# StefanDenn3r/Unsupervised_Anomaly_Detection_Brain_MRI

Measured on AMD Instinct MI355X. Metric: MRI slices/sec VAE train step (128x128, bs=64), higher is better.
Workload: dtype bf16x3; 1 GPU; BASELINE.json configs[1]: VAE 128x128x1 slices, batch 64 per GPU, fwd + bwd + TF-Adam (lr 1e-4, beta1 0.5), dropout 0.2, inter_res 8, zDim 128; global_batch=64, per_gpu_batch=64, parallelism=single

## Files before the change

include/uad_hip.h:

```cpp
#ifndef UAD_HIP_H
#define UAD_HIP_H

#include <stddef.h>
#include <stdint.h>

#ifdef __cplusplus
extern "C" {
#endif
#pragma GCC visibility push(default)

enum { UAD_OK = 0, UAD_ERR_INVALID = 1, UAD_ERR_HIP = 2, UAD_ERR_UNSUPPORTED = 3 };
enum { UAD_ARCH_AE = 0, UAD_ARCH_VAE = 1, UAD_ARCH_CEVAE = 2, UAD_ARCH_GMVAE_SPATIAL = 3,
       UAD_ARCH_AE_SPATIAL = 4 };
enum { UAD_BUF_PARAMS = 0, UAD_BUF_GRADS = 1, UAD_BUF_ADAM_M = 2, UAD_BUF_ADAM_V = 3 };
enum { UAD_SEG_DECODER = 0, UAD_SEG_BOTTLENECK = 1, UAD_SEG_ENCODER = 2, UAD_SEG_ENCODER_HI = 3, UAD_SEG_ENCODER_LO = 4, UAD_SEG_ALL = -1 };
enum { UAD_MATH_F32 = 0, UAD_MATH_BF16X3 = 1,
       UAD_MATH_BF16X3_ALL = 2 };
enum { UAD_MATH_BF16X6 = 3 };

typedef struct uad_model uad_model_t;

typedef struct {
    int arch;
    int height;
// ... 235 lines not shown
int uad_op_conv_w(const uad_conv_desc_t* d, const float* big, const uad_xform_t* xfb, const float* small_,
                  const uad_xform_t* xfs, float* dW, void* stream);
enum { UAD_OP_EPI_BIAS = 0, UAD_OP_EPI_BWD_ACT = 1, UAD_OP_EPI_FINAL = 2, UAD_OP_EPI_FINAL_TRAIN = 3, UAD_OP_EPI_FINAL_DC = 4 };
enum { UAD_OP_XF_IN = 1, UAD_OP_XF_SMALL = 2, UAD_OP_XF_FINAL_BWD = 4 };
int uad_op_conv_plan(const uad_conv_desc_t* d, int kind, int epi, int xf_flags, long long* out);
int uad_op_conv_d_final(const uad_conv_desc_t* d, const float* small_in, const uad_xform_t* xf, const float* W, const float* bias, const uad_xform_t* bn,
                        const float* wf, const float* bf, const float* x, float inv_batch, float* x_hat, float* l1, float* rec_sum,
                        unsigned* bits, float* dxhat, float* dc, float* red, void* stream);
int uad_op_conv_f_final_bwd(const uad_conv_desc_t* d, const unsigned* bits, const float* dxhat, const float* wf, const uad_xform_t* bn, const float* W,
                            const float* bias, const float* mul, const float* add, float* small_out, void* stream);
int uad_op_conv_first_fwd(const uad_conv_desc_t* d, const float* x, const float* W, const float* bias, float* out,
                          void* stream);
int uad_op_conv_first_wgrad(const uad_conv_desc_t* d, const float* x, const float* g, float* dW, void* stream);
int uad_op_adam(float* p, const float* g, float* m, float* v, long long n, float lr_t, float beta1, float beta2,
                float eps, float gscale, void* stream);

#pragma GCC visibility pop
#ifdef __cplusplus
}
#endif
#endif
```

unsupervised_anomaly_detection_brain_mri_amd/_lib.py:

```python
import ctypes as C
import os

_HERE = os.path.dirname(os.path.abspath(__file__))
LIB_PATH = os.environ.get('UAD_LIB') or os.path.join(_HERE, 'libuad_hip.so')

UAD_OK = 0
ARCH_AE, ARCH_VAE, ARCH_CEVAE, ARCH_GMVAE_SPATIAL, ARCH_AE_SPATIAL = 0, 1, 2, 3, 4
BUF_PARAMS, BUF_GRADS, BUF_ADAM_M, BUF_ADAM_V = 0, 1, 2, 3
SEG_DECODER, SEG_BOTTLENECK, SEG_ENCODER, SEG_ENCODER_HI, SEG_ENCODER_LO, SEG_ALL = 0, 1, 2, 3, 4, -1
MATH_F32, MATH_BF16X3, MATH_BF16X3_ALL, MATH_BF16X6 = 0, 1, 2, 3

c_float_p = C.c_void_p


class UadConfig(C.Structure):
    _fields_ = [('arch', C.c_int), ('height', C.c_int), ('width', C.c_int), ('channels', C.c_int),
                ('inter_res', C.c_int), ('zdim', C.c_int), ('max_batch', C.c_int),
                ('dim_c', C.c_int), ('dim_z', C.c_int), ('dim_w', C.c_int), ('c_lambda', C.c_float)]


class UadRngJob(C.Structure):
    _fields_ = [('out', C.c_void_p), ('per_sample', C.c_int), ('kind', C.c_int), ('rate', C.c_float), ('stream', C.c_int)]


# ... 31 lines not shown
HISTOGRAM_MAX_CLASSES, HISTOGRAM_SUM_CHAIN = 4, 1073
GAN_ENCODER, GAN_GENERATOR, GAN_DISCRIMINATOR = 0, 1, 2
GAN_UNIFIED, GAN_RESNET, GAN_ANOVAEGAN, GAN_AAE = 0, 1, 2, 3
GAN_GROUP_VAE = 3
BUF_ADAM_M2, BUF_ADAM_V2 = 4, 5
GAN_SCALARS = ('gen_loss', 'disc_fake', 'disc_real', 'penalty', 'disc_loss', 'loss_img', 'loss_fts', 'enc_loss',
               'reconstructionLoss', 'kl', 'gm_loss', 'gm_con', 'gm_w', 'gm_c')


class UadConvDesc(C.Structure):
    _fields_ = [(k, C.c_int) for k in ('N', 'HB', 'WB', 'CB', 'HS', 'WS', 'CS', 'KS', 'S', 'P')]


class UadXform(C.Structure):
    _fields_ = [('scale', C.c_void_p), ('shift', C.c_void_p), ('alpha', C.c_float)]


SYMBOLS = {
    'uad_last_error': (C.c_char_p, []),
    'uad_version': (C.c_char_p, []),
    'uad_create': (C.c_int, [C.POINTER(UadConfig), C.POINTER(C.c_void_p)]),
    'uad_destroy': (C.c_int, [C.c_void_p]),
    'uad_param_count': (C.c_longlong, [C.c_void_p]),
    'uad_num_tensors': (C.c_int, [C.c_void_p]),
    'uad_tensor_info': (C.c_int, [C.c_void_p, C.c_int, C.c_char_p, C.c_int, C.POINTER(C.c_longlong),
                                  C.POINTER(C.c_int), C.POINTER(C.c_int)]),
    'uad_buffer': (C.c_void_p, [C.c_void_p, C.c_int]),
    'uad_grad_segment': (C.c_int, [C.c_void_p, C.c_int, C.POINTER(C.c_longlong), C.POINTER(C.c_longlong)]),
    'uad_set_params': (C.c_int, [C.c_void_p, C.c_void_p, C.c_longlong]),
    'uad_get_params': (C.c_int, [C.c_void_p, C.c_void_p, C.c_longlong]),
# ... 103 lines not shown
    'uad_op_conv_d_bwdact': (C.c_int, [C.POINTER(UadConvDesc), C.c_void_p, C.c_void_p, C.c_void_p,
                                       C.POINTER(UadXform), C.c_void_p, C.c_void_p, C.c_void_p, C.c_void_p]),
    'uad_op_conv_w': (C.c_int, [C.POINTER(UadConvDesc), C.c_void_p, C.POINTER(UadXform), C.c_void_p,
                                C.POINTER(UadXform), C.c_void_p, C.c_void_p]),
    'uad_op_conv_plan': (C.c_int, [C.POINTER(UadConvDesc), C.c_int, C.c_int, C.c_int, C.POINTER(C.c_longlong)]),
    'uad_op_conv_d_final': (C.c_int, [C.POINTER(UadConvDesc), C.c_void_p, C.POINTER(UadXform), C.c_void_p, C.c_void_p, C.POINTER(UadXform),
                                      C.c_void_p, C.c_void_p, C.c_void_p, C.c_float, C.c_void_p, C.c_void_p, C.c_void_p,
                                      C.c_void_p, C.c_void_p, C.c_void_p, C.c_void_p, C.c_void_p]),
    'uad_op_conv_f_final_bwd': (C.c_int, [C.POINTER(UadConvDesc), C.c_void_p, C.c_void_p, C.c_void_p, C.POINTER(UadXform), C.c_void_p,
                                          C.c_void_p, C.c_void_p, C.c_void_p, C.c_void_p, C.c_void_p]),
    'uad_op_conv_first_fwd': (C.c_int, [C.POINTER(UadConvDesc), C.c_void_p, C.c_void_p, C.c_void_p, C.c_void_p,
                                        C.c_void_p]),
    'uad_op_conv_first_wgrad': (C.c_int, [C.POINTER(UadConvDesc), C.c_void_p, C.c_void_p, C.c_void_p, C.c_void_p]),
    'uad_op_adam': (C.c_int, [C.c_void_p, C.c_void_p, C.c_void_p, C.c_void_p, C.c_longlong, C.c_float, C.c_float,
                              C.c_float, C.c_float, C.c_float, C.c_void_p]),
}

_lib = None


def load():
    global _lib
    if _lib is not None:
        return _lib
    if not os.path.exists(LIB_PATH):
        raise RuntimeError(
            f'{LIB_PATH} is missing: the HIP extension has not been built '
            f'(run `python -m unsupervised_anomaly_detection_brain_mri_amd.build` or __graft_entry__.build()). '
            f'There is no CPU fallback.')
    import torch
# ... 16 lines not shown
```

unsupervised_anomaly_detection_brain_mri_amd/csrc/uad_conv_plan.hip:

```cpp
#include <stdint.h>
#include <stdio.h>
#include <stdlib.h>
#include <string.h>
#include "uad_conv_launch.h"
#include "uad_conv_k3_plan.h"

namespace {
thread_local bool g_any_order_next = false;
thread_local bool g_any_order_w_next = false;
inline bool take_request(bool& flag) { const bool on = flag; flag = false; return on; }

struct SpatialChoice { bool ok; int TH, TW, BN, CK; };
inline SpatialChoice choose_spatial(const UadConvDesc& d, int CA, int Nn, bool f_type = true) {
    SpatialChoice c{false, 0, 0, 0, 0};
    if (!(d.KS == 5 && d.S == 2 && d.P == 1)) return c;
    if (d.HB != 2 * d.HS || d.WB != 2 * d.WS) return c;
    if (CA > XF_LDS_CH) return c;
    if (Nn % 64 == 0 && CA % 32 == 0 && d.HS % 8 == 0 && d.WS % 8 == 0) { c = SpatialChoice{true, 8, 8, 64, 32}; return c; }
    if (Nn % 32 == 0 && CA % 16 == 0 && d.HS % 8 == 0 && d.WS % 16 == 0) {
        c = SpatialChoice{true, 8, 16, 32, (!f_type && CA % 32 == 0) ? 32 : 16};
        return c;
    }
    return c;
}
// ... 382 lines not shown
    a.lws = ilog2_exact(d.WS); a.lhs = ilog2_exact(d.HS); a.dbgbuf = nullptr;
    dim3 grid((a.Mtot + c.BM - 1) / c.BM, (d.CS + c.BN - 1) / c.BN, c.splits);
    static const bool w16_ok = !getenv("UAD_NO_W16");
    const bool w16 = generic_bf16x3 && w16_ok && !xfb.scale && !xfs.scale && c.BN == 64 && d.CB % 4 == 0 && d.CS % 4 == 0;
    uad_gemm_launch_w(a, grid, c.BM, c.BN, w16, st);
    if (c.splits > 1 && !defer_reduce) uad_launch_reduce_partials(partial, c.splits, a.Mtot * d.CS, 1.0f, dW, hop());
}

void uad_conv_any_order_next(bool on) { g_any_order_next = on; }
void uad_conv_w_any_order_next(bool on) { g_any_order_w_next = on; }
void uad_launch_conv_w_reduce(const UadConvDesc& d, float* dW, float* partial, hipStream_t st, bool math_bf16x3) {
    const W5Choice w5 = choose_w5(d, math_bf16x3);
    const int splits = w5.ok ? w5.splits : choose_w(d).splits;
    if (splits > 1) uad_launch_reduce_partials(partial, splits, d.KS * d.KS * d.CB * d.CS, 1.0f, dW, st);
}

void uad_conv_w_plan_query(const UadConvDesc& d, bool math_bf16x3, int planes16, bool fbb, bool xa, bool xs, bool generic_bf16x3, bool defer_reduce, long long* out) {
    const long long slab = (long long)d.KS * d.KS * d.CB * d.CS;
    out[5] = -1; out[6] = -1; out[9] = 0;
    const W5Choice w5 = choose_w5(d, math_bf16x3);
    if (w5.ok) {
        const bool use16 = w5_use16(math_bf16x3, planes16, fbb, xa, xs);
        out[0] = 1; out[1] = w5.splits; out[2] = (w5.total_tiles % w5.tiles_per_split) ? 1 : 0; out[3] = w5_ncsb(d, use16); out[4] = w5.total_tiles;
        if (math_bf16x3 && planes16 == 3) out[5] = use16 ? 1 : 0;
        out[7] = w5.tiles_per_split; out[8] = w5.splits > 1 ? w5.splits * slab : 0;
        return;
    }
    const WK3Choice k3 = choose_wk3(d);
    if (wk3_takes(k3, math_bf16x3 || generic_bf16x3, planes16, defer_reduce, fbb || xa || xs)) {
        out[0] = 2; out[1] = k3.splits; out[2] = (k3.total_tiles % k3.tiles_per_split) ? 1 : 0; out[3] = 0; out[4] = k3.total_tiles;
// ... 9 lines not shown
```

unsupervised_anomaly_detection_brain_mri_amd/csrc/uad_kernels.h:

```cpp
#pragma once
#include <stdint.h>
#ifndef UAD_HOST_EMULATION
#include <hip/hip_runtime.h>

int uad_fail(int code, const char* fmt, ...);
#define HIP_TRY(expr)                                                                                      \
    do {                                                                                                   \
        hipError_t e_ = (expr);                                                                            \
        if (e_ != hipSuccess) return uad_fail(UAD_ERR_HIP, "%s failed: %s", #expr, hipGetErrorString(e_)); \
    } while (0)

struct UadConvDesc {
    int N;
    int HB, WB, CB;
    int HS, WS, CS;
    int KS, S, P;
};

struct UadXform {
    const float* scale = nullptr;
    const float* shift = nullptr;
    float alpha = 1.f;
    float mult = 1.f;
    const float* fb_dxhat = nullptr;
// ... 63 lines not shown
bool uad_conv_d_x6_form_ok(const UadEpilogue& ep, bool has_xf);
void uad_conv_w_plan_query(const UadConvDesc& d, bool math_bf16x3, int planes16, bool fbb, bool xa, bool xs, bool generic_bf16x3, bool defer_reduce, long long* out);
size_t uad_conv_w_partial_floats(const UadConvDesc& d);
bool uad_conv_w_supports_fb_bits(const UadConvDesc& d, bool math_bf16x3);
void uad_launch_conv_w(const UadConvDesc& d, const float* big, UadXform xfb, const float* small, UadXform xfs,
                       float* dW, float* partial, hipStream_t st, bool math_bf16x3 = false,
                       hipStream_t reduce_st = nullptr, hipEvent_t ev = nullptr, bool generic_bf16x3 = false, bool defer_reduce = false, int planes16 = 2);
void uad_launch_conv_w_reduce(const UadConvDesc& d, float* dW, float* partial, hipStream_t st, bool math_bf16x3);

void uad_launch_reduce_partials(const float* partial, int S, int L, float scale, float* out, hipStream_t st);
void uad_launch_bn_grad_finalize(const float* colpart, int T, int C, const float* gamma, float rstd,
                                 float* dgamma, float* dbeta, float* dbias, hipStream_t st, float* scratch = nullptr);
size_t uad_bn_grad_finalize_scratch_floats(int C);
void uad_launch_final_gradfin(const float* red, int C, const float* gamma, float rstd, float* dwf, float* dbf, float* dgamma, float* dbeta,
                              float* dbias, hipStream_t st);
constexpr size_t kUadColsumScratchFloats = 64 * 1024;
void uad_launch_colsum(const float* g, int rows, int C, float* out, float* scratch, hipStream_t st);
size_t uad_colsum_scratch_floats(int rows, int C);

void uad_launch_conv_first_fwd(const UadConvDesc& d, const float* x, const float* W, const float* bias,
                               float* out, hipStream_t st);
size_t uad_conv_first_wgrad_partial_floats(const UadConvDesc& d);
void uad_launch_conv_first_wgrad(const UadConvDesc& d, const float* x, const float* g, float* dW,
                                 float* partial, hipStream_t st);

struct UadFinalArgs {
    int N, H, W, C;
    const float* c_last;
    const float* scale;
    const float* shift;
// ... 175 lines not shown
```

unsupervised_anomaly_detection_brain_mri_amd/csrc/uad_misc.hip:

```cpp
#include "uad_kernels.h"
#include <stdint.h>

namespace {

__device__ __forceinline__ float wave_sum(float v) {
#pragma unroll
    for (int o = 32; o > 0; o >>= 1) v += __shfl_xor(v, o);
    return v;
}

typedef float v4f_nt __attribute__((ext_vector_type(4)));
template <int JL, int SL>
__global__ void __launch_bounds__(JL * SL) reduce_partials4_kernel(const float* __restrict__ partial, int S, int L, float scale, float* __restrict__ out) {
    __shared__ v4f_nt red[SL][JL];
    const int jl = threadIdx.x % JL, sl = threadIdx.x / JL;
    const int j4 = blockIdx.x * JL + jl, L4 = L >> 2;
    v4f_nt a0 = {0.f, 0.f, 0.f, 0.f}, a1 = a0, a2 = a0, a3 = a0;
    if (j4 < L4) {
        const v4f_nt* p = reinterpret_cast<const v4f_nt*>(partial) + j4;
        int s = sl;
        for (; s + 3 * SL < S; s += 4 * SL) {
            const v4f_nt v0 = __builtin_nontemporal_load(p + (size_t)s * L4), v1 = __builtin_nontemporal_load(p + (size_t)(s + SL) * L4);
            const v4f_nt v2 = __builtin_nontemporal_load(p + (size_t)(s + 2 * SL) * L4), v3 = __builtin_nontemporal_load(p + (size_t)(s + 3 * SL) * L4);
            a0 += v0; a1 += v1; a2 += v2; a3 += v3;
        }
        for (; s < S; s += SL) a0 += __builtin_nontemporal_load(p + (size_t)s * L4);
    }
    red[sl][jl] = (a0 + a1) + (a2 + a3);
    __syncthreads();
    if (sl == 0 && j4 < L4) {
        v4f_nt t = red[0][jl];
#pragma unroll
        for (int k = 1; k < SL; ++k) t += red[k][jl];
        reinterpret_cast<v4f_nt*>(out)[j4] = t * scale;
    }
}

template <int SL>
__global__ void __launch_bounds__(64 * SL) reduce_partials_kernel(const float* __restrict__ partial, int S, int L,
                                                                  float scale, float* __restrict__ out, int nt) {
    __shared__ float red[SL][64];
    const int jl = threadIdx.x & 63, sl = threadIdx.x >> 6;
    const int j = blockIdx.x * 64 + jl;
    float a0 = 0.f, a1 = 0.f, a2 = 0.f, a3 = 0.f;
    if (j < L) {
        int s = sl;
        if (nt) {
            for (; s + 3 * SL < S; s += 4 * SL) {
                a0 += __builtin_nontemporal_load(partial + (size_t)s * L + j);
                a1 += __builtin_nontemporal_load(partial + (size_t)(s + SL) * L + j);
                a2 += __builtin_nontemporal_load(partial + (size_t)(s + 2 * SL) * L + j);
                a3 += __builtin_nontemporal_load(partial + (size_t)(s + 3 * SL) * L + j);
            }
        }
        for (; s + 3 * SL < S; s += 4 * SL) {
            a0 += partial[(size_t)s * L + j];
            a1 += partial[(size_t)(s + SL) * L + j];
            a2 += partial[(size_t)(s + 2 * SL) * L + j];
            a3 += partial[(size_t)(s + 3 * SL) * L + j];
        }
        for (; s < S; s += SL) a0 += partial[(size_t)s * L + j];
    }
    red[sl][jl] = (a0 + a1) + (a2 + a3);
    __syncthreads();
    if (sl == 0 && j < L) {
        float t = 0.f;
#pragma unroll
        for (int k = 0; k < SL; ++k) t += red[k][jl];
        out[j] = t * scale;
    }
}

__global__ void __launch_bounds__(1024) bn_grad_finalize_kernel(const float* __restrict__ colpart, int T, int C,
                                                                const float* __restrict__ gamma, float rstd,
                                                                float* __restrict__ dgamma, float* __restrict__ dbeta,
                                                                float* __restrict__ dbias) {
    __shared__ float red[2][32][33];
    const int cl = threadIdx.x & 31, g = threadIdx.x >> 5;
    const int c = blockIdx.x * 32 + cl;
    float s1 = 0.f, s2 = 0.f;
    if (c < C) {
        for (int t = g; t < T; t += 32) {
            s1 += colpart[((size_t)t * 2 + 0) * C + c];
            s2 += colpart[((size_t)t * 2 + 1) * C + c];
        }
// ... 54 lines not shown
        if (dbias) dbias[c] = gamma[c] * rstd * a1;
    }
}

__global__ void __launch_bounds__(256) final_gradfin_kernel(const float* __restrict__ red, int C, const float* __restrict__ gamma, float rstd,
                                                            float* __restrict__ dwf, float* __restrict__ dbf, float* __restrict__ dgamma,
                                                            float* __restrict__ dbeta, float* __restrict__ dbias) {
    for (int c = threadIdx.x; c < C; c += 256) {
        const float s1 = red[C + c], s2 = red[2 * C + c];
        dwf[c] = red[c];
        if (dbeta) dbeta[c] = s1;
        if (dgamma) dgamma[c] = s2 * rstd;
        if (dbias) dbias[c] = gamma[c] * rstd * s1;
    }
    if (threadIdx.x == 0) dbf[0] = red[3 * C];
}

__global__ void __launch_bounds__(256) colsum_kernel(const float* __restrict__ g, int rows, int C, int rows_per_chunk,
                                                     float* __restrict__ out) {
    __shared__ float red[8][33];
    const int cl = threadIdx.x & 31, rl = threadIdx.x >> 5;
    const int c = blockIdx.x * 32 + cl;
    const int r0 = blockIdx.y * rows_per_chunk;
    const int r1 = min(r0 + rows_per_chunk, rows);
    float s = 0.f;
    if (c < C)
        for (int r = r0 + rl; r < r1; r += 8) s += g[(size_t)r * C + c];
    red[rl][cl] = s;
    __syncthreads();
    if (rl == 0 && c < C) {
// ... 758 lines not shown
}
void uad_launch_clock_probe(unsigned long long* out, unsigned long long ticks, hipStream_t st) {
    hipLaunchKernelGGL(clock_probe_kernel, dim3(1), dim3(64), 0, st, out, ticks);
}

void uad_launch_gather_slices(const float* src, const int* idx, int n, long long slice_elems, float* out, hipStream_t st) {
    const long long f4 = slice_elems / 4;
    int bx = (int)((f4 + 255) / 256); if (bx > 64) bx = 64; if (bx < 1) bx = 1;
    hipLaunchKernelGGL(gather_slices_kernel, dim3(bx, n), dim3(256), 0, st, src, idx, f4, out);
}
void uad_launch_gather_mask(const unsigned char* labels, const int* idx, int n, long long slice_px, const unsigned char* lut,
                            float* out, hipStream_t st) {
    int bx = (int)((slice_px + 255) / 256); if (bx > 64) bx = 64; if (bx < 1) bx = 1;
    hipLaunchKernelGGL(gather_mask_kernel, dim3(bx, n), dim3(256), 0, st, labels, idx, slice_px, lut, out);
}
void uad_launch_reduce_partials(const float* partial, int S, int L, float scale, float* out, hipStream_t st) {
    const int blocks = (L + 63) / 64;
    constexpr int nt = 1;
    static const bool r4 = getenv("UAD_NO_REDUCE4") == nullptr;
    if (r4 && S > 8 && L % 4 == 0 && L >= 1024 && ((uintptr_t)partial & 15) == 0 && ((uintptr_t)out & 15) == 0) {
        const int L4 = L / 4;
        if ((L4 + 63) / 64 >= 256) hipLaunchKernelGGL((reduce_partials4_kernel<64, 8>), dim3((L4 + 63) / 64), dim3(512), 0, st, partial, S, L, scale, out);
        else if ((L4 + 31) / 32 >= 256) hipLaunchKernelGGL((reduce_partials4_kernel<32, 16>), dim3((L4 + 31) / 32), dim3(512), 0, st, partial, S, L, scale, out);
        else hipLaunchKernelGGL((reduce_partials4_kernel<16, 32>), dim3((L4 + 15) / 16), dim3(512), 0, st, partial, S, L, scale, out);
        return;
    }
    if (blocks >= 256 || S <= 8)
        hipLaunchKernelGGL((reduce_partials_kernel<4>), dim3(blocks), dim3(256), 0, st, partial, S, L, scale, out, nt);
    else
        hipLaunchKernelGGL((reduce_partials_kernel<16>), dim3(blocks), dim3(1024), 0, st, partial, S, L, scale, out, nt);
}

void uad_launch_final_gradfin(const float* red, int C, const float* gamma, float rstd, float* dwf, float* dbf, float* dgamma, float* dbeta,
                              float* dbias, hipStream_t st) {
    hipLaunchKernelGGL(final_gradfin_kernel, dim3(1), dim3(256), 0, st, red, C, gamma, rstd, dwf, dbf, dgamma, dbeta, dbias);
}
size_t uad_bn_grad_finalize_scratch_floats(int C) { return 64 + (size_t)((C + 31) / 32) * 32 * 64; }
void uad_launch_bn_grad_finalize(const float* colpart, int T, int C, const float* gamma, float rstd, float* dgamma,
                                 float* dbeta, float* dbias, hipStream_t st, float* scratch) {
    const int NB = T >= 2048 ? 32 : T >= 512 ? 16 : T >= 128 ? 8 : 1;
    if (scratch && NB > 1 && C <= 512) {
        hipLaunchKernelGGL(bn_grad_finalize2_kernel, dim3((C + 31) / 32, NB), dim3(1024), 0, st, colpart, T, C, gamma, rstd, dgamma, dbeta, dbias, scratch);
        return;
    }
    hipLaunchKernelGGL(bn_grad_finalize_kernel, dim3((C + 31) / 32), dim3(1024), 0, st, colpart, T, C, gamma, rstd,
// ... 168 lines not shown
```

unsupervised_anomaly_detection_brain_mri_amd/csrc/uad_model.hip:

```cpp
#include <math.h>
#include <stdio.h>
#include <string.h>
#include <stdlib.h>

#include <string>
#include <vector>

#include <unistd.h>
#include "uad_handle.h"

namespace {

struct ConvLayer {
    UadConvDesc d;
    long long w, b, gamma, beta;
    float* c;
};

}

struct uad_model : UadHandleCore {
    uad_config_t cfg;
    int n_pool, cenc, cmid, flat;
    long long seg_off[5], seg_cnt[5];
// ... 346 lines not shown
    m->dec_in0 = (gm || sp) ? m->gm_h : m->cb;
    ALLOC(m->G0, maxact); ALLOC(m->G1, maxact);
    { float* fbw = nullptr; ALLOC(fbw, NB * H * Wd); m->fin_bits = reinterpret_cast<unsigned*>(fbw); ALLOC(m->fin_dxh, NB * H * Wd); }
    m->last_fin_bits = false;
    ALLOC(m->g_small[0], nflat); ALLOC(m->g_small[1], nz); ALLOC(m->g_small[2], nz); ALLOC(m->g_small[3], nz);
    ALLOC(m->g_small[4], nflat); ALLOC(m->g_small[5], nflat);
    ALLOC(m->dcb_keep, NB * ir * ir * m->cenc);
    ALLOC(m->bott_xch, NB * 4 * 2 * (size_t)cfg->zdim);
    { float* fl = nullptr; ALLOC(fl, NB * 4); m->bott_flags = reinterpret_cast<unsigned*>(fl); m->bott_epoch = 0; }
    m->bott_err_host = m->bott_err_dev = nullptr;
    { float* fw = nullptr; ALLOC(fw, 4); m->bott_fault = reinterpret_cast<unsigned*>(fw); m->opt_epochs.clear(); m->fault_deferred = false; }
    if (rc == UAD_OK && hipHostMalloc((void**)&m->bott_err_host, sizeof(unsigned), hipHostMallocMapped) == hipSuccess) {
        *m->bott_err_host = 0u;
        if (hipHostGetDevicePointer((void**)&m->bott_err_dev, m->bott_err_host, 0) != hipSuccess) m->bott_err_dev = nullptr;
    }
    ALLOC(m->bnfin_scratch, uad_bn_grad_finalize_scratch_floats(512));
    ALLOC(m->bott_wpart, NB * 4 * (2 * (size_t)m->cenc * m->cmid + m->cmid));
    size_t cp = 0;
    auto cp_need = [&](size_t rows, int classes, int C) { size_t v = ((rows + 63) / 64) * classes * 2 * C; if (v > cp) cp = v; };
    for (auto& L : m->enc) cp_need(NB * L.d.HS * L.d.WS, 4, L.d.CB);
    for (auto& L : m->dec) cp_need(NB * L.d.HS * L.d.WS, 1, L.d.CS);
    cp_need(NB * ir * ir, 1, m->cenc);
    if (NB * 4 * 2 * m->cenc > cp) cp = NB * 4 * 2 * m->cenc;
    if (gm) { size_t v = NB * ir * ir * 2 * m->cenc; if (v > cp) cp = v; }
    if (sp) { size_t v = (size_t)512 * 2 * m->cenc; if (v > cp) cp = v; }
    m->colpart_cap = cp; ALLOC(m->colpart, cp);
    for (int k = 0; k < 16; ++k) { m->cp_slot[k] = nullptr; ALLOC(m->cp_slot[k], cp); }
    m->ev_next = 0; m->side = nullptr;
    if (rc == UAD_OK && hipStreamCreateWithFlags(&m->side, hipStreamNonBlocking) != hipSuccess) rc = fail(UAD_ERR_HIP, "hipStreamCreate failed");
    size_t wp = 0;
    auto wp_need = [&](UadConvDesc d) { for (size_t nb = m->nmul; nb <= NB; nb += m->nmul) { d.N = (int)nb; size_t v = uad_conv_w_partial_floats(d); if (v > wp) wp = v; } };
// ... 380 lines not shown
    if (m->ev_next == m->sync_events.size()) {
        hipEvent_t e;
        if (hipEventCreateWithFlags(&e, hipEventDisableTiming | hipEventDisableSystemFence) != hipSuccess)
            (void)hipEventCreateWithFlags(&e, hipEventDisableTiming);
        m->sync_events.push_back(e);
    }
    return m->sync_events[m->ev_next++];
}
static void edge(uad_model* m, hipStream_t from, hipStream_t to) {
    hipEvent_t e = next_event(m);
    (void)hipEventRecord(e, from);
    (void)hipStreamWaitEvent(to, e, 0);
}
#define PROF_ON(tag, stream) ProfScope prof_scope_s_##__LINE__(m, tag, stream)
static void join_side(uad_model* m, hipStream_t st) { edge(m, m->side, st); m->joined = true; }

static int backward_decoder(uad_model* m, hipStream_t st, bool join_now) {
    const int n = m->last_n;
    const float rstd = 1.0f / sqrtf(1.0f + kBnEps);
    hipStream_t sd = m->side;
    const bool bf = bf_mode(m);
    const ConvLayer& DL = m->dec.back();
    const int C = DL.d.CB;
    const int bps = uad_final_blocks_per_sample(m->cfg.height, m->cfg.width);
    const int T = n * bps, L = 3 * C + 1;
    static const char* kDecW[] = {"dec0.wgrad", "dec1.wgrad", "dec2.wgrad", "dec3.wgrad", "dec4.wgrad", "dec5.wgrad", "dec6.wgrad", "dec7.wgrad"};
    static const char* kDecD[] = {"dec0.dgrad", "dec1.dgrad", "dec2.dgrad", "dec3.dgrad", "dec4.dgrad", "dec5.dgrad", "dec6.dgrad", "dec7.dgrad"};
    const bool pg = !m->data_only;
    m->ev_next = 0;
    float* g = m->G0;
// ... 10 lines not shown
        const bool fbb = last && m->last_fin_bits;
        UadXform gbits = no_xform();
        if (fbb) { gbits = bn_xform(m, DL.gamma, DL.beta, kLrelu); gbits.fb_dxhat = m->restore ? m->gm_dxhat : m->fin_dxh; gbits.fb_wf = P(m, m->fw); gbits.fb_bits = m->fin_bits; }
        { static const bool anyo = getenv("UAD_NO_ANYORDER") == nullptr;
          if (anyo && pg && bf && last && m->fwd_tail_is_loss && !m->prof_on) uad_conv_w_any_order_next(true);
          m->fwd_tail_is_loss = false; }
        if (pg) { PROF(kDecW[i & 7]); uad_launch_conv_w(d, g, fbb ? gbits : no_xform(), in, bn_xform(m, ig, ib, ia), Gr(m, m->dec[i].w), m->wp_slot[i], st, bf, nullptr, nullptr, false, true, planes_of(m)); }
        uad_conv_w_any_order_next(false);
        { static const bool anyo = getenv("UAD_NO_ANYORDER") == nullptr; if (anyo && pg) uad_conv_any_order_next(true); }
        { PROF(kDecD[i & 7]); UadEpilogue e = epi_bwd(m, in, ig, ib, ia); e.colpart = cp;
          const bool fb = m->restore && m->fb_on_load && last;
          UadXform gx = fbb ? gbits : no_xform();
          if (fb) { gx = bn_xform(m, DL.gamma, DL.beta, kLrelu); gx.fb_dxhat = m->gm_dxhat; gx.fb_wf = P(m, m->fw); }
          uad_launch_conv_f(d, fb ? DL.c : g, gx, P(m, m->dec[i].w), gn, e, st, PKF(m, m->dec[i].w), m->ws, PK16F(m, m->dec[i].w), PLANE(m->dec[i]), false, planes_of(m));
          uad_conv_any_order_next(false); }
        if (pg) edge(m, st, sd);
        if (pg && last) {
            PROF_ON("final.gradfin", sd);
            uad_launch_reduce_partials(m->red_partial, T, L, 1.0f, m->colscratch, sd);
            uad_launch_final_gradfin(m->colscratch, C, P(m, DL.gamma), rstd, Gr(m, m->fw), Gr(m, m->fb), Gr(m, DL.gamma), Gr(m, DL.beta), Gr(m, DL.b), sd);
        }
        if (pg) { PROF_ON("bn.gradfin", sd); uad_launch_conv_w_reduce(d, Gr(m, m->dec[i].w), m->wp_slot[i], sd, bf); uad_launch_bn_grad_finalize(cp, uad_conv_f_tiles(d, true, m->ws.floats, sk_counters(m), planes_of(m)), d.CS, P(m, ig), rstd, Gr(m, ig), Gr(m, ib), ibias >= 0 ? Gr(m, ibias) : nullptr, sd, m->bnfin_scratch); }
        float* tsw = g; g = gn; gn = tsw;
    }
    m->G0 = g; m->G1 = gn;
    if (join_now) join_side(m, st);
    return UAD_OK;
}

static int backward_bottleneck(uad_model* m, hipStream_t st, bool join_now) {
// ... 157 lines not shown
    const bool bf = bf_mode(m);
    const bool pg = !m->data_only;
    float* g = m->G0;
    float* gn = m->G1;
    static const char* kEncW[] = {"enc0.wgrad", "enc1.wgrad", "enc2.wgrad", "enc3.wgrad", "enc4.wgrad", "enc5.wgrad", "enc6.wgrad", "enc7.wgrad"};
    static const char* kEncD[] = {"enc0.dgrad", "enc1.dgrad", "enc2.dgrad", "enc3.dgrad", "enc4.dgrad", "enc5.dgrad", "enc6.dgrad", "enc7.dgrad"};
    const int hi_from = (int)m->enc.size() - 1, hi_to = m->enc.size() >= 3 ? 2 : hi_from + 1;
    const int i_first = part == 2 ? hi_to - 1 : hi_from, i_last = part == 1 ? hi_to : 1;
    for (int i = i_first; i >= i_last; --i) {
        UadConvDesc d = m->enc[i].d; d.N = n;
        const ConvLayer& PL = m->enc[i - 1];
        float* cp = m->cp_slot[8 + (i & 7)];
        if (pg) { PROF(kEncW[i & 7]); uad_launch_conv_w(d, PL.c, bn_xform(m, PL.gamma, PL.beta, kLrelu), g, no_xform(), Gr(m, m->enc[i].w), m->wp_slot[8 + (i & 7)], st, bf, nullptr, nullptr, false, true, planes_of(m)); }
        static const bool tail_split_on = getenv("UAD_NO_TAIL_SPLIT") == nullptr;
        const bool tail_split = tail_split_on && pg && part != 1 && i == i_last && !m->prof_on;
        if (tail_split) { edge(m, st, sd); PROF_ON("bn.gradfin", sd); uad_launch_conv_w_reduce(d, Gr(m, m->enc[i].w), m->wp_slot[8 + (i & 7)], sd, bf); }
        { static const bool anyo = getenv("UAD_NO_ANYORDER") == nullptr; if (anyo && pg) uad_conv_any_order_next(true); }
        { PROF(kEncD[i & 7]); UadEpilogue e = epi_bwd(m, PL.c, PL.gamma, PL.beta, kLrelu); e.colpart = cp;
          uad_launch_conv_d(d, g, no_xform(), P(m, m->enc[i].w), gn, e, st, PKD(m, m->enc[i].w), m->ws, PK16D(m, m->enc[i].w), PLANE(m->enc[i]), false, planes_of(m));
          uad_conv_any_order_next(false); }
        if (pg) edge(m, st, sd);
        if (pg) { PROF_ON("bn.gradfin", sd); if (!tail_split) uad_launch_conv_w_reduce(d, Gr(m, m->enc[i].w), m->wp_slot[8 + (i & 7)], sd, bf);
                  uad_launch_bn_grad_finalize(cp, uad_conv_d_tiles(d, true, m->ws.floats, sk_counters(m), planes_of(m)), d.CB, P(m, PL.gamma), rstd, Gr(m, PL.gamma),
                                    Gr(m, PL.beta), Gr(m, PL.b), sd, m->bnfin_scratch); }
        float* tsw = g; g = gn; gn = tsw;
    }
    if (part == 1) {
        m->G0 = g; m->G1 = gn;
        if (!defer) join_side(m, st);
        return UAD_OK;
    }
    UadConvDesc d0 = m->enc[0].d; d0.N = n;
    if (pg) { PROF("enc0.wgrad"); uad_launch_conv_first_wgrad(d0, m->x_eff, g, Gr(m, m->enc[0].w), m->wp_slot[8], st); }
    if (m->restore && (m->restore_x || m->restore_grads)) {
        PROF("enc0.dgrad");
// ... 272 lines not shown
```

unsupervised_anomaly_detection_brain_mri_amd/csrc/uad_ops.hip:

```cpp
#include <stdarg.h>
#include <stdio.h>
#include <stdlib.h>
#include <string.h>

#include <string>

#include "uad_handle.h"

static thread_local std::string g_err;

int uad_fail(int code, const char* fmt, ...) {
    char buf[512];
    va_list ap;
    va_start(ap, fmt);
    vsnprintf(buf, sizeof buf, fmt, ap);
    va_end(ap);
    g_err = buf;
    return code;
}

extern "C" {

const char* uad_last_error(void) { return g_err.c_str(); }
const char* uad_version(void) { return "uad_hip 0.1 (gfx950, fp32 MFMA)"; }
// ... 311 lines not shown
    HIP_TRY(hipMalloc((void**)&partial, uad_conv_first_wgrad_partial_floats(d) * sizeof(float)));
    hipStream_t st = (hipStream_t)stream;
    uad_launch_conv_first_wgrad(d, x, g, dW, partial, st);
    HIP_TRY(hipStreamSynchronize(st));
    hipFree(partial);
    HIP_TRY(hipGetLastError());
    return UAD_OK;
}
int uad_op_adam(float* p, const float* g, float* mm, float* v, long long n, float lr_t, float beta1, float beta2, float eps,
                float gscale, void* stream) {
    uad_launch_adam(p, g, mm, v, (size_t)n, lr_t, beta1, beta2, eps, gscale, (hipStream_t)stream);
    HIP_TRY(hipGetLastError());
    return UAD_OK;
}

}
```

Baseline: 78700 slices/s.

## Fuse weight-grad reduce, BN grad finalize and final gradfin into one side-stream kernel

```diff
diff --git a/include/uad_hip.h b/include/uad_hip.h
--- a/include/uad_hip.h
+++ b/include/uad_hip.h
@@ -273,6 +273,13 @@
 int uad_op_conv_first_wgrad(const uad_conv_desc_t* d, const float* x, const float* g, float* dW, void* stream);
 int uad_op_adam(float* p, const float* g, float* m, float* v, long long n, float lr_t, float beta1, float beta2,
                 float eps, float gscale, void* stream);
+typedef struct {
+    const float* slabs; int S, L; float* dW;
+    const float* colpart; int T, C; const float* gamma; float rstd; float *dgamma, *dbeta, *dbias;
+    const float* fin_partial; int fin_T, fin_C; const float* fin_gamma; float *dwf, *dbf, *fin_dgamma, *fin_dbeta, *fin_dbias, *fin_red;
+} uad_grad_finish_t;
+long long uad_op_grad_finish_scratch_floats(void);
+int uad_op_grad_finish(const uad_grad_finish_t* a, int fused, float* scratch, void* stream);
 
 #pragma GCC visibility pop
 #ifdef __cplusplus
diff --git a/unsupervised_anomaly_detection_brain_mri_amd/_lib.py b/unsupervised_anomaly_detection_brain_mri_amd/_lib.py
--- a/unsupervised_anomaly_detection_brain_mri_amd/_lib.py
+++ b/unsupervised_anomaly_detection_brain_mri_amd/_lib.py
@@ -69,6 +69,15 @@
 
 class UadXform(C.Structure):
     _fields_ = [('scale', C.c_void_p), ('shift', C.c_void_p), ('alpha', C.c_float)]
+
+
+class UadGradFinish(C.Structure):
+    _fields_ = [('slabs', C.c_void_p), ('S', C.c_int), ('L', C.c_int), ('dW', C.c_void_p),
+                ('colpart', C.c_void_p), ('T', C.c_int), ('C', C.c_int), ('gamma', C.c_void_p), ('rstd', C.c_float),
+                ('dgamma', C.c_void_p), ('dbeta', C.c_void_p), ('dbias', C.c_void_p),
+                ('fin_partial', C.c_void_p), ('fin_T', C.c_int), ('fin_C', C.c_int), ('fin_gamma', C.c_void_p),
+                ('dwf', C.c_void_p), ('dbf', C.c_void_p), ('fin_dgamma', C.c_void_p), ('fin_dbeta', C.c_void_p), ('fin_dbias', C.c_void_p),
+                ('fin_red', C.c_void_p)]
 
 
 SYMBOLS = {
@@ -202,6 +211,8 @@
     'uad_op_conv_first_wgrad': (C.c_int, [C.POINTER(UadConvDesc), C.c_void_p, C.c_void_p, C.c_void_p, C.c_void_p]),
     'uad_op_adam': (C.c_int, [C.c_void_p, C.c_void_p, C.c_void_p, C.c_void_p, C.c_longlong, C.c_float, C.c_float,
                               C.c_float, C.c_float, C.c_float, C.c_void_p]),
+    'uad_op_grad_finish_scratch_floats': (C.c_longlong, []),
+    'uad_op_grad_finish': (C.c_int, [C.POINTER(UadGradFinish), C.c_int, C.c_void_p, C.c_void_p]),
 }
 
 _lib = None
diff --git a/unsupervised_anomaly_detection_brain_mri_amd/csrc/uad_conv_plan.hip b/unsupervised_anomaly_detection_brain_mri_amd/csrc/uad_conv_plan.hip
--- a/unsupervised_anomaly_detection_brain_mri_amd/csrc/uad_conv_plan.hip
+++ b/unsupervised_anomaly_detection_brain_mri_amd/csrc/uad_conv_plan.hip
@@ -420,6 +420,12 @@
     const int splits = w5.ok ? w5.splits : choose_w(d).splits;
     if (splits > 1) uad_launch_reduce_partials(partial, splits, d.KS * d.KS * d.CB * d.CS, 1.0f, dW, st);
 }
+void uad_launch_conv_w_finish(const UadConvDesc& d, float* dW, float* partial, bool math_bf16x3, UadGradFinish a, hipStream_t st) {
+    const W5Choice w5 = choose_w5(d, math_bf16x3);
+    const int splits = w5.ok ? w5.splits : choose_w(d).splits;
+    a.partial = splits > 1 ? partial : nullptr; a.S = splits > 1 ? splits : 0; a.L = d.KS * d.KS * d.CB * d.CS; a.dW = dW;
+    uad_launch_grad_finish(a, st);
+}
 
 void uad_conv_w_plan_query(const UadConvDesc& d, bool math_bf16x3, int planes16, bool fbb, bool xa, bool xs, bool generic_bf16x3, bool defer_reduce, long long* out) {
     const long long slab = (long long)d.KS * d.KS * d.CB * d.CS;
diff --git a/unsupervised_anomaly_detection_brain_mri_amd/csrc/uad_kernels.h b/unsupervised_anomaly_detection_brain_mri_amd/csrc/uad_kernels.h
--- a/unsupervised_anomaly_detection_brain_mri_amd/csrc/uad_kernels.h
+++ b/unsupervised_anomaly_detection_brain_mri_amd/csrc/uad_kernels.h
@@ -101,6 +101,17 @@
 size_t uad_bn_grad_finalize_scratch_floats(int C);
 void uad_launch_final_gradfin(const float* red, int C, const float* gamma, float rstd, float* dwf, float* dbf, float* dgamma, float* dbeta,
                               float* dbias, hipStream_t st);
+struct UadGradFinish {
+    const float* partial; int S, L; float* dW;
+    const float* colpart; int T, C; const float* gamma; float rstd; float *dgamma, *dbeta, *dbias;
+    const float* fin_partial; int fin_T, fin_C; const float* fin_gamma; float *dwf, *dbf, *fin_dgamma, *fin_dbeta, *fin_dbias;
+    float* scratch;
+    int nfin, nbn, NB;
+};
+bool uad_grad_finish_takes(int C, int fin_C);
+size_t uad_grad_finish_scratch_floats();
+void uad_launch_grad_finish(const UadGradFinish& a, hipStream_t st);
+void uad_launch_conv_w_finish(const UadConvDesc& d, float* dW, float* partial, bool math_bf16x3, UadGradFinish a, hipStream_t st);
 constexpr size_t kUadColsumScratchFloats = 64 * 1024;
 void uad_launch_colsum(const float* g, int rows, int C, float* out, float* scratch, hipStream_t st);
 size_t uad_colsum_scratch_floats(int rows, int C);
diff --git a/unsupervised_anomaly_detection_brain_mri_amd/csrc/uad_misc.hip b/unsupervised_anomaly_detection_brain_mri_amd/csrc/uad_misc.hip
--- a/unsupervised_anomaly_detection_brain_mri_amd/csrc/uad_misc.hip
+++ b/unsupervised_anomaly_detection_brain_mri_amd/csrc/uad_misc.hip
@@ -11,10 +11,9 @@
 
 typedef float v4f_nt __attribute__((ext_vector_type(4)));
 template <int JL, int SL>
-__global__ void __launch_bounds__(JL * SL) reduce_partials4_kernel(const float* __restrict__ partial, int S, int L, float scale, float* __restrict__ out) {
-    __shared__ v4f_nt red[SL][JL];
+__device__ __forceinline__ void reduce4_block(v4f_nt (*red)[JL], int vb, const float* __restrict__ partial, int S, int L, float scale, float* __restrict__ out) {
     const int jl = threadIdx.x % JL, sl = threadIdx.x / JL;
-    const int j4 = blockIdx.x * JL + jl, L4 = L >> 2;
+    const int j4 = vb * JL + jl, L4 = L >> 2;
     v4f_nt a0 = {0.f, 0.f, 0.f, 0.f}, a1 = a0, a2 = a0, a3 = a0;
     if (j4 < L4) {
         const v4f_nt* p = reinterpret_cast<const v4f_nt*>(partial) + j4;
@@ -35,13 +34,17 @@
         reinterpret_cast<v4f_nt*>(out)[j4] = t * scale;
     }
 }
-
-template <int SL>
-__global__ void __launch_bounds__(64 * SL) reduce_partials_kernel(const float* __restrict__ partial, int S, int L,
-                                                                  float scale, float* __restrict__ out, int nt) {
-    __shared__ float red[SL][64];
-    const int jl = threadIdx.x & 63, sl = threadIdx.x >> 6;
-    const int j = blockIdx.x * 64 + jl;
+template <int JL, int SL>
+__global__ void __launch_bounds__(JL * SL) reduce_partials4_kernel(const float* __restrict__ partial, int S, int L, float scale, float* __restrict__ out) {
+    __shared__ v4f_nt red[SL][JL];
+    reduce4_block<JL, SL>(red, blockIdx.x, partial, S, L, scale, out);
+}
+
+template <int JL, int SL>
+__device__ __forceinline__ void reduce1_block(float (*red)[JL], int vb, const float* __restrict__ partial, int S, int L,
+                                              float scale, float* __restrict__ out, int nt) {
+    const int jl = threadIdx.x % JL, sl = threadIdx.x / JL;
+    const int j = vb * JL + jl;
     float a0 = 0.f, a1 = 0.f, a2 = 0.f, a3 = 0.f;
     if (j < L) {
         int s = sl;
@@ -69,6 +72,12 @@
         for (int k = 0; k < SL; ++k) t += red[k][jl];
         out[j] = t * scale;
     }
+}
+template <int SL>
+__global__ void __launch_bounds__(64 * SL) reduce_partials_kernel(const float* __restrict__ partial, int S, int L,
+                                                                  float scale, float* __restrict__ out, int nt) {
+    __shared__ float red[SL][64];
+    reduce1_block<64, SL>(red, blockIdx.x, partial, S, L, scale, out, nt);
 }
 
 __global__ void __launch_bounds__(1024) bn_grad_finalize_kernel(const float* __restrict__ colpart, int T, int C,
@@ -153,6 +162,131 @@
         if (dbias) dbias[c] = gamma[c] * rstd * s1;
     }
     if (threadIdx.x == 0) dbf[0] = red[3 * C];
+}
+
+constexpr int kFinishBnFloats = 64 + 16 * 32 * 64;
+constexpr int kFinishFinCounter = 32;
+constexpr int kFinishFinCols = 256;
+
+__device__ __forceinline__ void finish_bn_block(const UadGradFinish& a, int v, float* lds, int* s_last) {
+    float (*red)[32][33] = reinterpret_cast<float (*)[32][33]>(lds);
+    const int CG = (a.C + 31) >> 5, NB = a.NB, C = a.C;
+    const int bx = v % CG, by = v / CG;
+    const int cl = threadIdx.x & 31, g = threadIdx.x >> 5;
+    const int c = bx * 32 + cl;
+    const int tper = (a.T + NB - 1) / NB, t0 = by * tper, t1 = min(t0 + tper, a.T);
+    float s1 = 0.f, s2 = 0.f, u1 = 0.f, u2 = 0.f;
+    if (c < C) {
+        int t = t0 + g;
+        for (; t + 16 < t1; t += 32) {
+            s1 += a.colpart[((size_t)t * 2 + 0) * C + c];
+            s2 += a.colpart[((size_t)t * 2 + 1) * C + c];
+            u1 += a.colpart[((size_t)(t + 16) * 2 + 0) * C + c];
+            u2 += a.colpart[((size_t)(t + 16) * 2 + 1) * C + c];
+        }
+        if (t < t1) {
+            s1 += a.colpart[((size_t)t * 2 + 0) * C + c];
+            s2 += a.colpart[((size_t)t * 2 + 1) * C + c];
+        }
+    }
+    red[0][g][cl] = s1; red[0][g + 16][cl] = u1;
+    red[1][g][cl] = s2; red[1][g + 16][cl] = u2;
+    __syncthreads();
+    if (NB == 1) {
+        if (g == 0 && c < C) {
+            float a1 = 0.f, a2 = 0.f;
+            for (int k = 0; k < 32; ++k) { a1 += red[0][k][cl]; a2 += red[1][k][cl]; }
+            if (a.dbeta) a.dbeta[c] = a1;
+            if (a.dgamma) a.dgamma[c] = a2 * a.rstd;
+            if (a.dbias) a.dbias[c] = a.gamma[c] * a.rstd * a1;
+        }
+        return;
+    }
+    unsigned* cnt = reinterpret_cast<unsigned*>(a.scratch) + bx;
+    float* part = a.scratch + 64 + ((size_t)bx * NB) * 64;
+    if (g < 2) {
+        float s = 0.f;
+        for (int k = 0; k < 32; ++k) s += red[g][k][cl];
+        __hip_atomic_store(part + by * 64 + g * 32 + cl, s, __ATOMIC_RELAXED, __HIP_MEMORY_SCOPE_AGENT);
+        __builtin_amdgcn_s_waitcnt(0);
+    }
+    __builtin_amdgcn_fence(__ATOMIC_RELEASE, "workgroup");
+    __syncthreads();
+    if (threadIdx.x == 0) *s_last = (__hip_atomic_fetch_add(cnt, 1u, __ATOMIC_RELAXED, __HIP_MEMORY_SCOPE_AGENT) == (unsigned)(NB - 1));
+    __syncthreads();
+    if (!*s_last) return;
+    if (threadIdx.x == 0) __hip_atomic_store(cnt, 0u, __ATOMIC_RELAXED, __HIP_MEMORY_SCOPE_AGENT);
+    if (g == 0 && c < C) {
+        float a1 = 0.f, a2 = 0.f;
+        for (int k = 0; k < NB; ++k) {
+            a1 += __hip_atomic_load(part + k * 64 + cl, __ATOMIC_RELAXED, __HIP_MEMORY_SCOPE_AGENT);
+            a2 += __hip_atomic_load(part + k * 64 + 32 + cl, __ATOMIC_RELAXED, __HIP_MEMORY_SCOPE_AGENT);
+        }
+        if (a.dbeta) a.dbeta[c] = a1;
+        if (a.dgamma) a.dgamma[c] = a2 * a.rstd;
+        if (a.dbias) a.dbias[c] = a.gamma[c] * a.rstd * a1;
+    }
+}
+
+__device__ __forceinline__ void finish_final_block(const UadGradFinish& a, int f, float* lds, int* s_last) {
+    float (*ch)[kFinishFinCols] = reinterpret_cast<float (*)[kFinishFinCols]>(lds);
+    float* sums = lds + 4 * kFinishFinCols;
+    const int SL = a.nfin, S = a.fin_T, C = a.fin_C, L = 3 * C + 1;
+    const int tid = threadIdx.x, jl = tid & 127, k = tid >> 7;
+    const float* __restrict__ p = a.fin_partial;
+    for (int j = jl; j < kFinishFinCols; j += 128) {
+        float acc = 0.f;
+        if (j < L) {
+            int s = f;
+#pragma unroll 4
+            for (; s + 3 * SL < S; s += 4 * SL) acc += p[(size_t)(s + k * SL) * L + j];
+            if (k == 0) for (; s < S; s += SL) acc += p[(size_t)s * L + j];
+        }
+        ch[k][j] = acc;
+    }
+    __syncthreads();
+    unsigned* cnt = reinterpret_cast<unsigned*>(a.scratch) + kFinishFinCounter;
+    float* part = a.scratch + kFinishBnFloats;
+    if (tid < L) {
+        __hip_atomic_store(part + f * kFinishFinCols + tid, (ch[0][tid] + ch[1][tid]) + (ch[2][tid] + ch[3][tid]), __ATOMIC_RELAXED, __HIP_MEMORY_SCOPE_AGENT);
+        __builtin_amdgcn_s_waitcnt(0);
+    }
+    __builtin_amdgcn_fence(__ATOMIC_RELEASE, "workgroup");
+    __syncthreads();
+    if (tid == 0) *s_last = (__hip_atomic_fetch_add(cnt, 1u, __ATOMIC_RELAXED, __HIP_MEMORY_SCOPE_AGENT) == (unsigned)(SL - 1));
+    __syncthreads();
+    if (!*s_last) return;
+    if (tid == 0) __hip_atomic_store(cnt, 0u, __ATOMIC_RELAXED, __HIP_MEMORY_SCOPE_AGENT);
+    if (tid < L) {
+        float t = 0.f;
+        for (int q = 0; q < SL; ++q) t += __hip_atomic_load(part + q * kFinishFinCols + tid, __ATOMIC_RELAXED, __HIP_MEMORY_SCOPE_AGENT);
+        sums[tid] = t;
+    }
+    __syncthreads();
+    for (int c = tid; c < C; c += 512) {
+        const float s1 = sums[C + c], s2 = sums[2 * C + c];
+        a.dwf[c] = sums[c];
+        if (a.fin_dbeta) a.fin_dbeta[c] = s1;
+        if (a.fin_dgamma) a.fin_dgamma[c] = s2 * a.rstd;
+        if (a.fin_dbias) a.fin_dbias[c] = a.fin_gamma[c] * a.rstd * s1;
+    }
+    if (tid == 0) a.dbf[0] = sums[3 * C];
+}
+
+enum { RF_NONE = 0, RF_VEC64, RF_VEC32, RF_VEC16, RF_SCALAR4, RF_SCALAR16 };
+template <int SLAB>
+__global__ void __launch_bounds__(512) grad_finish_kernel(const UadGradFinish a) {
+    __shared__ __attribute__((aligned(16))) float lds[2 * 32 * 33];
+    __shared__ int s_last;
+    const int b = blockIdx.x;
+    if (b < a.nfin) { finish_final_block(a, b, lds, &s_last); return; }
+    if (b < a.nfin + a.nbn) { finish_bn_block(a, b - a.nfin, lds, &s_last); return; }
+    const int vb = b - a.nfin - a.nbn;
+    if constexpr (SLAB == RF_VEC64) reduce4_block<64, 8>(reinterpret_cast<v4f_nt (*)[64]>(lds), vb, a.partial, a.S, a.L, 1.0f, a.dW);
+    else if constexpr (SLAB == RF_VEC32) reduce4_block<32, 16>(reinterpret_cast<v4f_nt (*)[32]>(lds), vb, a.partial, a.S, a.L, 1.0f, a.dW);
+    else if constexpr (SLAB == RF_VEC16) reduce4_block<16, 32>(reinterpret_cast<v4f_nt (*)[16]>(lds), vb, a.partial, a.S, a.L, 1.0f, a.dW);
+    else if constexpr (SLAB == RF_SCALAR4) reduce1_block<128, 4>(reinterpret_cast<float (*)[128]>(lds), vb, a.partial, a.S, a.L, 1.0f, a.dW, 1);
+    else if constexpr (SLAB == RF_SCALAR16) reduce1_block<32, 16>(reinterpret_cast<float (*)[32]>(lds), vb, a.partial, a.S, a.L, 1.0f, a.dW, 1);
 }
 
 __global__ void __launch_bounds__(256) colsum_kernel(const float* __restrict__ g, int rows, int C, int rows_per_chunk,
@@ -941,21 +1075,50 @@
     int bx = (int)((slice_px + 255) / 256); if (bx > 64) bx = 64; if (bx < 1) bx = 1;
     hipLaunchKernelGGL(gather_mask_kernel, dim3(bx, n), dim3(256), 0, st, labels, idx, slice_px, lut, out);
 }
-void uad_launch_reduce_partials(const float* partial, int S, int L, float scale, float* out, hipStream_t st) {
-    const int blocks = (L + 63) / 64;
-    constexpr int nt = 1;
+static int reduce_form(const float* partial, int S, int L, const float* out) {
     static const bool r4 = getenv("UAD_NO_REDUCE4") == nullptr;
     if (r4 && S > 8 && L % 4 == 0 && L >= 1024 && ((uintptr_t)partial & 15) == 0 && ((uintptr_t)out & 15) == 0) {
         const int L4 = L / 4;
-        if ((L4 + 63) / 64 >= 256) hipLaunchKernelGGL((reduce_partials4_kernel<64, 8>), dim3((L4 + 63) / 64), dim3(512), 0, st, partial, S, L, scale, out);
-        else if ((L4 + 31) / 32 >= 256) hipLaunchKernelGGL((reduce_partials4_kernel<32, 16>), dim3((L4 + 31) / 32), dim3(512), 0, st, partial, S, L, scale, out);
-        else hipLaunchKernelGGL((reduce_partials4_kernel<16, 32>), dim3((L4 + 15) / 16), dim3(512), 0, st, partial, S, L, scale, out);
-        return;
-    }
-    if (blocks >= 256 || S <= 8)
-        hipLaunchKernelGGL((reduce_partials_kernel<4>), dim3(blocks), dim3(256), 0, st, partial, S, L, scale, out, nt);
-    else
-        hipLaunchKernelGGL((reduce_partials_kernel<16>), dim3(blocks), dim3(1024), 0, st, partial, S, L, scale, out, nt);
+        return (L4 + 63) / 64 >= 256 ? RF_VEC64 : (L4 + 31) / 32 >= 256 ? RF_VEC32 : RF_VEC16;
+    }
+    return ((L + 63) / 64 >= 256 || S <= 8) ? RF_SCALAR4 : RF_SCALAR16;
+}
+void uad_launch_reduce_partials(const float* partial, int S, int L, float scale, float* out, hipStream_t st) {
+    const int blocks = (L + 63) / 64, L4 = L / 4;
+    constexpr int nt = 1;
+    switch (reduce_form(partial, S, L, out)) {
+    case RF_VEC64: hipLaunchKernelGGL((reduce_partials4_kernel<64, 8>), dim3((L4 + 63) / 64), dim3(512), 0, st, partial, S, L, scale, out); break;
+    case RF_VEC32: hipLaunchKernelGGL((reduce_partials4_kernel<32, 16>), dim3((L4 + 31) / 32), dim3(512), 0, st, partial, S, L, scale, out); break;
+    case RF_VEC16: hipLaunchKernelGGL((reduce_partials4_kernel<16, 32>), dim3((L4 + 15) / 16), dim3(512), 0, st, partial, S, L, scale, out); break;
+    case RF_SCALAR4: hipLaunchKernelGGL((reduce_partials_kernel<4>), dim3(blocks), dim3(256), 0, st, partial, S, L, scale, out, nt); break;
+    default: hipLaunchKernelGGL((reduce_partials_kernel<16>), dim3(blocks), dim3(1024), 0, st, partial, S, L, scale, out, nt); break;
+    }
+}
+
+bool uad_grad_finish_takes(int C, int fin_C) { return C <= 512 && 3 * fin_C + 1 <= kFinishFinCols; }
+size_t uad_grad_finish_scratch_floats() { return (size_t)kFinishBnFloats + 16 * kFinishFinCols; }
+void uad_launch_grad_finish(const UadGradFinish& in, hipStream_t st) {
+    UadGradFinish a = in;
+    if (!a.fin_partial) a.fin_C = 0;
+    if (!a.colpart) a.C = 0;
+    if (!uad_grad_finish_takes(a.C, a.fin_C)) { fprintf(stderr, "uad: grad_finish does not take C = %d, fin_C = %d (uad_grad_finish_takes)\n", a.C, a.fin_C); abort(); }
+    a.nfin = a.fin_partial ? (a.fin_T <= 8 ? 4 : 16) : 0;
+    a.NB = a.T >= 2048 ? 32 : a.T >= 512 ? 16 : a.T >= 128 ? 8 : 1;
+    a.nbn = a.colpart ? ((a.C + 31) / 32) * a.NB : 0;
+    const int form = (a.partial && a.S > 0) ? reduce_form(a.partial, a.S, a.L, a.dW) : RF_NONE;
+    const int L4 = a.L / 4;
+    const int nslab = form == RF_VEC64 ? (L4 + 63) / 64 : form == RF_VEC32 ? (L4 + 31) / 32 : form == RF_VEC16 ? (L4 + 15) / 16
+                      : form == RF_SCALAR4 ? (a.L + 127) / 128 : form == RF_SCALAR16 ? (a.L + 31) / 32 : 0;
+    const dim3 grid(a.nfin + a.nbn + nslab);
+    if (!grid.x) return;
+    switch (form) {
+    case RF_VEC64: hipLaunchKernelGGL(grad_finish_kernel<RF_VEC64>, grid, dim3(512), 0, st, a); break;
+    case RF_VEC32: hipLaunchKernelGGL(grad_finish_kernel<RF_VEC32>, grid, dim3(512), 0, st, a); break;
+    case RF_VEC16: hipLaunchKernelGGL(grad_finish_kernel<RF_VEC16>, grid, dim3(512), 0, st, a); break;
+    case RF_SCALAR4: hipLaunchKernelGGL(grad_finish_kernel<RF_SCALAR4>, grid, dim3(512), 0, st, a); break;
+    case RF_SCALAR16: hipLaunchKernelGGL(grad_finish_kernel<RF_SCALAR16>, grid, dim3(512), 0, st, a); break;
+    default: hipLaunchKernelGGL(grad_finish_kernel<RF_NONE>, grid, dim3(512), 0, st, a); break;
+    }
 }
 
 void uad_launch_final_gradfin(const float* red, int C, const float* gamma, float rstd, float* dwf, float* dbf, float* dgamma, float* dbeta,
diff --git a/unsupervised_anomaly_detection_brain_mri_amd/csrc/uad_model.hip b/unsupervised_anomaly_detection_brain_mri_amd/csrc/uad_model.hip
--- a/unsupervised_anomaly_detection_brain_mri_amd/csrc/uad_model.hip
+++ b/unsupervised_anomaly_detection_brain_mri_amd/csrc/uad_model.hip
@@ -384,7 +384,7 @@
         *m->bott_err_host = 0u;
         if (hipHostGetDevicePointer((void**)&m->bott_err_dev, m->bott_err_host, 0) != hipSuccess) m->bott_err_dev = nullptr;
     }
-    ALLOC(m->bnfin_scratch, uad_bn_grad_finalize_scratch_floats(512));
+    ALLOC(m->bnfin_scratch, uad_grad_finish_scratch_floats());
     ALLOC(m->bott_wpart, NB * 4 * (2 * (size_t)m->cenc * m->cmid + m->cmid));
     size_t cp = 0;
     auto cp_need = [&](size_t rows, int classes, int C) { size_t v = ((rows + 63) / 64) * classes * 2 * C; if (v > cp) cp = v; };
@@ -795,6 +795,19 @@
 }
 #define PROF_ON(tag, stream) ProfScope prof_scope_s_##__LINE__(m, tag, stream)
 static void join_side(uad_model* m, hipStream_t st) { edge(m, m->side, st); m->joined = true; }
+
+static bool side_fuse(const uad_model* m, int C, int fin_C) {
+    static const bool on = getenv("UAD_NO_SIDE_FUSE") == nullptr;
+    return on && bf_mode(m) && uad_grad_finish_takes(C, fin_C);
+}
+static UadGradFinish bn_finish(uad_model* m, const float* cp, int T, int C, long long gamma, long long beta, long long bias) {
+    UadGradFinish f;
+    memset(&f, 0, sizeof f);
+    f.colpart = cp; f.T = T; f.C = C; f.gamma = P(m, gamma); f.rstd = 1.0f / sqrtf(1.0f + kBnEps);
+    f.dgamma = Gr(m, gamma); f.dbeta = Gr(m, beta); f.dbias = bias >= 0 ? Gr(m, bias) : nullptr;
+    f.scratch = m->bnfin_scratch;
+    return f;
+}
 
 static int backward_decoder(uad_model* m, hipStream_t st, bool join_now) {
     const int n = m->last_n;
@@ -835,6 +848,19 @@
           if (fb) { gx = bn_xform(m, DL.gamma, DL.beta, kLrelu); gx.fb_dxhat = m->gm_dxhat; gx.fb_wf = P(m, m->fw); }
           uad_launch_conv_f(d, fb ? DL.c : g, gx, P(m, m->dec[i].w), gn, e, st, PKF(m, m->dec[i].w), m->ws, PK16F(m, m->dec[i].w), PLANE(m->dec[i]), false, planes_of(m));
           uad_conv_any_order_next(false); }
+        if (pg && side_fuse(m, d.CS, last ? C : 0)) {
+            UadGradFinish f = bn_finish(m, cp, uad_conv_f_tiles(d, true, m->ws.floats, sk_counters(m), planes_of(m)), d.CS, ig, ib, ibias);
+            UadGradFinish ff = f;
+            ff.colpart = nullptr; ff.fin_partial = m->red_partial; ff.fin_T = T; ff.fin_C = C; ff.fin_gamma = P(m, DL.gamma);
+            ff.dwf = Gr(m, m->fw); ff.dbf = Gr(m, m->fb); ff.fin_dgamma = Gr(m, DL.gamma); ff.fin_dbeta = Gr(m, DL.beta); ff.fin_dbias = Gr(m, DL.b);
+            if (last && !m->prof_on) { ff.colpart = f.colpart; f = ff; }
+            edge(m, st, sd);
+            if (last && m->prof_on) { PROF_ON("final.gradfin", sd); ff.partial = nullptr; uad_launch_grad_finish(ff, sd); }
+            PROF_ON("bn.gradfin", sd);
+            uad_launch_conv_w_finish(d, Gr(m, m->dec[i].w), m->wp_slot[i], bf, f, sd);
+            float* tsw = g; g = gn; gn = tsw;
+            continue;
+        }
         if (pg) edge(m, st, sd);
         if (pg && last) {
             PROF_ON("final.gradfin", sd);
@@ -1022,11 +1048,24 @@
         if (pg) { PROF(kEncW[i & 7]); uad_launch_conv_w(d, PL.c, bn_xform(m, PL.gamma, PL.beta, kLrelu), g, no_xform(), Gr(m, m->enc[i].w), m->wp_slot[8 + (i & 7)], st, bf, nullptr, nullptr, false, true, planes_of(m)); }
         static const bool tail_split_on = getenv("UAD_NO_TAIL_SPLIT") == nullptr;
         const bool tail_split = tail_split_on && pg && part != 1 && i == i_last && !m->prof_on;
-        if (tail_split) { edge(m, st, sd); PROF_ON("bn.gradfin", sd); uad_launch_conv_w_reduce(d, Gr(m, m->enc[i].w), m->wp_slot[8 + (i & 7)], sd, bf); }
+        const bool fuse = pg && side_fuse(m, d.CB, 0);
+        if (tail_split) {
+            edge(m, st, sd); PROF_ON("bn.gradfin", sd);
+            uad_launch_conv_w_reduce(d, Gr(m, m->enc[i].w), m->wp_slot[8 + (i & 7)], sd, bf);
+        }
         { static const bool anyo = getenv("UAD_NO_ANYORDER") == nullptr; if (anyo && pg) uad_conv_any_order_next(true); }
         { PROF(kEncD[i & 7]); UadEpilogue e = epi_bwd(m, PL.c, PL.gamma, PL.beta, kLrelu); e.colpart = cp;
           uad_launch_conv_d(d, g, no_xform(), P(m, m->enc[i].w), gn, e, st, PKD(m, m->enc[i].w), m->ws, PK16D(m, m->enc[i].w), PLANE(m->enc[i]), false, planes_of(m));
           uad_conv_any_order_next(false); }
+        if (fuse) {
+            const UadGradFinish f = bn_finish(m, cp, uad_conv_d_tiles(d, true, m->ws.floats, sk_counters(m), planes_of(m)), d.CB, PL.gamma, PL.beta, PL.b);
+            edge(m, st, sd);
+            PROF_ON("bn.gradfin", sd);
+            if (tail_split) uad_launch_grad_finish(f, sd);
+            else uad_launch_conv_w_finish(d, Gr(m, m->enc[i].w), m->wp_slot[8 + (i & 7)], bf, f, sd);
+            float* tsw = g; g = gn; gn = tsw;
+            continue;
+        }
         if (pg) edge(m, st, sd);
         if (pg) { PROF_ON("bn.gradfin", sd); if (!tail_split) uad_launch_conv_w_reduce(d, Gr(m, m->enc[i].w), m->wp_slot[8 + (i & 7)], sd, bf);
                   uad_launch_bn_grad_finalize(cp, uad_conv_d_tiles(d, true, m->ws.floats, sk_counters(m), planes_of(m)), d.CB, P(m, PL.gamma), rstd, Gr(m, PL.gamma),
diff --git a/unsupervised_anomaly_detection_brain_mri_amd/csrc/uad_ops.hip b/unsupervised_anomaly_detection_brain_mri_amd/csrc/uad_ops.hip
--- a/unsupervised_anomaly_detection_brain_mri_amd/csrc/uad_ops.hip
+++ b/unsupervised_anomaly_detection_brain_mri_amd/csrc/uad_ops.hip
@@ -349,4 +349,33 @@
     return UAD_OK;
 }
 
-}
+long long uad_op_grad_finish_scratch_floats(void) { return (long long)uad_grad_finish_scratch_floats(); }
+int uad_op_grad_finish(const uad_grad_finish_t* a, int fused, float* scratch, void* stream) {
+    if (!a || !scratch) return fail(UAD_ERR_INVALID, "grad_finish: null argument");
+    if ((a->slabs && (a->S < 1 || a->L < 1 || !a->dW)) || (a->colpart && (a->T < 1 || a->C < 1 || !a->gamma)) ||
+        (a->fin_partial && (a->fin_T < 1 || a->fin_C < 1 || !a->fin_gamma || !a->dwf || !a->dbf || !a->fin_red)))
+        return fail(UAD_ERR_INVALID, "grad_finish: a part with an input needs its sizes and outputs");
+    hipStream_t st = (hipStream_t)stream;
+    if (fused) {
+        if (!uad_grad_finish_takes(a->colpart ? a->C : 0, a->fin_partial ? a->fin_C : 0)) return fail(UAD_ERR_UNSUPPORTED, "grad_finish: C <= 512 and fin_C <= 64 in one launch");
+        UadGradFinish f;
+        memset(&f, 0, sizeof f);
+        f.partial = a->slabs; f.S = a->S; f.L = a->L; f.dW = a->dW;
+        f.colpart = a->colpart; f.T = a->T; f.C = a->C; f.gamma = a->gamma; f.rstd = a->rstd; f.dgamma = a->dgamma; f.dbeta = a->dbeta; f.dbias = a->dbias;
+        f.fin_partial = a->fin_partial; f.fin_T = a->fin_T; f.fin_C = a->fin_C; f.fin_gamma = a->fin_gamma;
+        f.dwf = a->dwf; f.dbf = a->dbf; f.fin_dgamma = a->fin_dgamma; f.fin_dbeta = a->fin_dbeta; f.fin_dbias = a->fin_dbias;
+        f.scratch = scratch;
+        uad_launch_grad_finish(f, st);
+    } else {
+        if (a->fin_partial) {
+            uad_launch_reduce_partials(a->fin_partial, a->fin_T, 3 * a->fin_C + 1, 1.0f, a->fin_red, st);
+            uad_launch_final_gradfin(a->fin_red, a->fin_C, a->fin_gamma, a->rstd, a->dwf, a->dbf, a->fin_dgamma, a->fin_dbeta, a->fin_dbias, st);
+        }
+        if (a->slabs) uad_launch_reduce_partials(a->slabs, a->S, a->L, 1.0f, a->dW, st);
+        if (a->colpart) uad_launch_bn_grad_finalize(a->colpart, a->T, a->C, a->gamma, a->rstd, a->dgamma, a->dbeta, a->dbias, st, scratch);
+    }
+    HIP_TRY(hipGetLastError());
+    return UAD_OK;
+}
+
+}
```

Measured after the change: 79910 slices/s, median of 6. +1.5%, better.
